# zzz5y/street_crafter

Measured on AMD Instinct MI355X. Metric: frames/sec @1M Gaussians 1920x1280 + PSNR vs ref; 1/2/4/8 MI355X, higher is better.
Workload: dtype f32

## Files before the change

### include/street_crafter_amd.h

```cpp
#ifndef STREET_CRAFTER_AMD_H
#define STREET_CRAFTER_AMD_H

#include <stddef.h>
#include <stdint.h>

#ifdef __cplusplus
extern "C" {
#endif

typedef void* sc_stream_t;

#define SC_OK 0
#define SC_EINVAL (-1)
#define SC_EWORKSPACE (-2)
#define SC_EUNSUPPORTED (-3)

const char* sc_version(void);
const char* sc_error_string(int code);
const char* sc_target_arch(void);
int sc_wait_i64(const int64_t* addr, int64_t value, int64_t timeout_us);

int sc_projection_fwd(const float* means, const float* quats, const float* scales,
                      const float* viewmats, const float* Ks, int C, int N, int width, int height,
                      float eps2d, float near_plane, float far_plane, float radius_clip,
// ... 42 lines not shown
int64_t sc_isect_split_seg_bound(int64_t n_records, int nsb);
int sc_isect_split_bins(const uint64_t* keys, int64_t n, uint64_t lo, uint64_t hi, int32_t* bins);
int sc_isect_split_plan(const uint32_t* bin_counts, int cap, int32_t* range_of_bin, int32_t* n_ranges);
int sc_isect_bin_sort(const float* means2d, const int32_t* radii, const float* depths, int C, int N,
                      int tile_size, int tile_width, int tile_height,
                      const int32_t* isect_offsets, const int64_t* meta_dev,
                      void* count_workspace ,
                      int64_t capacity, int64_t rec_capacity, int64_t super_capacity,
                      int64_t* isect_ids , int32_t* flatten_ids,
                      void* workspace, size_t ws_bytes, sc_stream_t stream);
int sc_isect_ids_rebuild(const int32_t* flatten_ids, const int32_t* isect_offsets, const float* depths,
                         int C, int N, int tile_width, int tile_height, int64_t n_isects,
                         int64_t* isect_ids, sc_stream_t stream);
int sc_isect_bin_reset_cursors(void* count_workspace, int64_t CN, int C, int tile_width, int tile_height,
                               sc_stream_t stream);

int sc_isect_offsets(const int64_t* isect_ids, int64_t n_isects, int C, int tile_width,
                     int tile_height, int32_t* offsets, sc_stream_t stream);

int sc_sh_fwd(int degree, const float* dirs, const float* coeffs, const uint8_t* masks,
              int64_t M, int K, float* colors, sc_stream_t stream);
int sc_sh_bwd(int degree, const float* dirs, const float* coeffs, const uint8_t* masks,
              int64_t M, int K, const float* v_colors, float* v_coeffs, float* v_dirs,
              sc_stream_t stream);

int sc_rasterize_fwd(const float* means2d, const float* conics, const float* colors,
                     const float* opacities, const float* backgrounds, const uint8_t* tile_masks,
                     int C, int N, int D, int width, int height, int tile_size,
                     int tile_width, int tile_height,
                     const int32_t* isect_offsets, const int32_t* flatten_ids, int64_t n_isects,
// ... 349 lines not shown
```

### street_crafter_amd/_lib.py

```python
from __future__ import annotations

import ctypes as C
import os

_HERE = os.path.dirname(os.path.abspath(__file__))
LIB_PATH = os.path.join(_HERE, "lib", "libstreet_crafter_hip.so")
DIAG_LIB_PATH = os.path.join(_HERE, "lib", "libstreet_crafter_hip_diag.so")

_lib = None
_path = LIB_PATH
_lock = __import__("threading").Lock()


def use_diagnostic_build(tag: str = ""):
    global _path
    want = DIAG_LIB_PATH.replace("_diag.so", f"_diag_{tag}.so") if tag else DIAG_LIB_PATH
    if _lib is not None and _path != want:
        raise RuntimeError("use_diagnostic_build() must be called before the library is first loaded")
    if not os.path.exists(want):
        raise ImportError(f"diagnostic library not built ({want} missing): "
                          "python -m street_crafter_amd.build --diag")
    _path = want

c_f32p = C.c_void_p
# ... 74 lines not shown
                                     c_i32p, c_i64p, c_i64p, C.c_int64, C.c_void_p, C.c_size_t, c_i32p, c_f32p, c_i32p,
                                     c_i32p, c_stream]),
    "sc_view_slots": (C.c_int, []),
    "sc_view_registry_words": (C.c_int, []),
    "sc_isect_bin_bucket_capacity": (C.c_int, []),
    "sc_isect_split_limits": (C.c_int, [c_i64p]),
    "sc_isect_split_seg_bound": (C.c_int64, [C.c_int64, C.c_int]),
    "sc_isect_split_bins": (C.c_int, [c_u64p, C.c_int64, C.c_uint64, C.c_uint64, c_i32p]),
    "sc_isect_split_plan": (C.c_int, [C.c_void_p, C.c_int, c_i32p, c_i32p]),
    "sc_isect_bin_sort": (C.c_int, [c_f32p, c_i32p, c_f32p, C.c_int, C.c_int, C.c_int, C.c_int, C.c_int,
                                    c_i32p, c_i64p, C.c_void_p, C.c_int64, C.c_int64, C.c_int64, c_i64p,
                                    c_i32p, C.c_void_p, C.c_size_t, c_stream]),
    "sc_isect_ids_rebuild": (C.c_int, [c_i32p, c_i32p, c_f32p, C.c_int, C.c_int, C.c_int, C.c_int, C.c_int64, c_i64p,
                                       c_stream]),
    "sc_isect_bin_reset_cursors": (C.c_int, [C.c_void_p, C.c_int64, C.c_int, C.c_int, C.c_int, c_stream]),
    "sc_isect_offsets": (C.c_int, [c_i64p, C.c_int64, C.c_int, C.c_int, C.c_int, c_i32p, c_stream]),
    "sc_sh_fwd": (C.c_int, [C.c_int, c_f32p, c_f32p, c_u8p, C.c_int64, C.c_int, c_f32p, c_stream]),
    "sc_sh_bwd": (C.c_int, [C.c_int, c_f32p, c_f32p, c_u8p, C.c_int64, C.c_int, c_f32p, c_f32p, c_f32p,
                            c_stream]),
    "sc_rasterize_fwd": (C.c_int, [c_f32p, c_f32p, c_f32p, c_f32p, c_f32p, c_u8p, C.c_int, C.c_int, C.c_int,
                                   C.c_int, C.c_int, C.c_int, C.c_int, C.c_int, c_i32p, c_i32p, C.c_int64,
                                   c_f32p, c_f32p, c_i32p, c_i32p, c_i32p, c_stream]),
    "sc_rasterize_fwd_ed": (C.c_int, [c_f32p, c_f32p, c_f32p, c_f32p, c_f32p, c_u8p, C.c_int, C.c_int, C.c_int,
                                      C.c_int, C.c_int, C.c_int, C.c_int, C.c_int, c_i32p, c_i32p, C.c_int64,
                                      c_f32p, c_f32p, c_i32p, c_i32p, c_stream]),
    "sc_rasterize_fwd_planar": (C.c_int, [c_f32p, c_f32p, c_f32p, c_f32p, c_f32p, c_u8p, C.c_int, C.c_int, C.c_int,
                                          C.c_int, C.c_int, C.c_int, C.c_int, C.c_int, c_i32p, c_i32p, C.c_int64,
                                          c_f32p, c_f32p, c_i32p, c_i32p, c_stream]),
    "sc_group_extents": (C.c_int, [c_i32p, c_i32p, C.c_int64, c_u8p, C.c_int, C.c_int, C.c_int, C.c_int, C.c_int,
                                   c_i32p, c_stream]),
# ... 135 lines not shown
    lib = C.CDLL(_path)
    for name, (res, args) in SIGNATURES.items():
        fn = getattr(lib, name)
        fn.restype = res
        fn.argtypes = args
    _lib = lib
    env_c, env_f = os.environ.get("SC_PROJ_CLAMP"), os.environ.get("SC_RADIUS_FLOOR")
    if env_c:
        if env_c not in ("symmetric", "asymmetric"):
            raise ValueError(f"SC_PROJ_CLAMP must be symmetric or asymmetric, got {env_c!r}")
        lib.sc_set_option(b"proj_clamp", 1 if env_c == "asymmetric" else 0)
    if env_f:
        if float(env_f) not in (0.01, 0.1):
            raise ValueError(f"SC_RADIUS_FLOOR must be 0.01 or 0.1, got {env_f!r}")
        lib.sc_set_option(b"radius_floor", 1 if float(env_f) == 0.1 else 0)
    return lib


FAST_PATH = os.path.join(_HERE, "lib", "_sc_fast.so")
_fast = None
_fast_enabled = True


def fast():
    global _fast
    if not _fast_enabled or _path != LIB_PATH:
        return None
    if _fast is None:
        load()
        with _lock:
# ... 65 lines not shown
```

### street_crafter_amd/csrc/capi.hip

```cpp
#include "raster_common.h"
#include <string.h>
#include <time.h>

#ifndef SC_ABI_HASH
#define SC_ABI_HASH "unhashed"
#endif
#ifdef SC_DIAG
extern "C" const char* sc_version(void) { return "street_crafter_amd 0.4.0 (gfx950, DIAGNOSTIC build) abi:" SC_ABI_HASH; }
#else
extern "C" const char* sc_version(void) { return "street_crafter_amd 0.4.0 (gfx950) abi:" SC_ABI_HASH; }
#endif

extern "C" const char* sc_target_arch(void) { return "gfx950"; }

extern "C" const char* sc_error_string(int code) {
    switch (code) {
        case SC_OK: return "ok";
        case SC_EINVAL: return "street_crafter_amd: invalid argument (size / null pointer / unsupported parameter)";
        case SC_EWORKSPACE: return "street_crafter_amd: workspace too small";
        case SC_EUNSUPPORTED: return "street_crafter_amd: unsupported configuration";
        default: break;
    }
    if (code > 0) return hipGetErrorString((hipError_t)code);
    return "street_crafter_amd: unknown error";
// ... 76 lines not shown
        if (value < 0 || value > 1) return SC_EINVAL;
        const int prev = g_sc_raster_map;
        g_sc_raster_map = value;
        return prev;
    }
    if (strcmp(key, "raster_hint_blend") == 0) {
        if (value < 0 || value > 4) return SC_EINVAL;
        const int prev = g_sc_raster_hint_blend;
        g_sc_raster_hint_blend = value;
        return prev;
    }
    if (strcmp(key, "raster_split") == 0) {
        if (value < 0 || value > 100) return SC_EINVAL;
        const int prev = g_sc_raster_split;
        g_sc_raster_split = value;
        return prev;
    }
    if (strcmp(key, "proj_clamp") == 0) {
        if (value < 0 || value > 1) return SC_EINVAL;
        const int prev = g_sc_proj_clamp;
        g_sc_proj_clamp = value;
        return prev;
    }
    if (strcmp(key, "radius_floor") == 0) {
        if (value < 0 || value > 1) return SC_EINVAL;
        const int prev = g_sc_radius_floor;
        g_sc_radius_floor = value;
        return prev;
    }
    if (strcmp(key, "point_raster_waves") == 0) {
// ... 232 lines not shown
```

### street_crafter_amd/csrc/isect_bin.hip

```cpp
#include "sc_common.h"

#pragma clang fp contract(off)

#include "isect_split_plan.h"

namespace {

constexpr int BIN_THREADS = 1024;
constexpr int BIN_GPT = 4;
constexpr int BIN_GPB = BIN_THREADS * BIN_GPT;
constexpr int CNT_GPT = 8;
constexpr int BIN_MAX_TILES = 36864;
constexpr int BIN_BIG = 32;
constexpr unsigned ID_MASK = 0x0fffffffu;
constexpr unsigned long long KEY_MASK = 0xffffffff0fffffffull;

struct Rect { int x0, x1, y0, y1; };

struct Geo {
    int tile_width, tile_height, T;
    int ss;
    int stw, sth, ST;
    int N;
};
// ... 405 lines not shown
        return;
    }
    const int cblock = (int)blockIdx.x - 3;
    unsigned* hist = lds;
    unsigned* gbase = lds + n_sbuckets;
    unsigned* cst = lds + 2 * n_sbuckets;
    {
        const int per = (n_sbuckets + BIN_THREADS - 1) / BIN_THREADS;
        const int beg = min((int)threadIdx.x * per, n_sbuckets), end = min(beg + per, n_sbuckets);
        long long sum = 0;
        for (int i = beg; i < end; ++i) sum += chist[i];
        long long tot;
        unsigned mx;
        long long run = block_scan_1024(sum, 0u, &tot, &mx, wave_tot, wave_max);
        for (int i = beg; i < end; ++i) { cst[i] = (unsigned)run; run += chist[i]; }
        if (cblock == 0 && threadIdx.x == 0) { cmeta[0] = tot; cmeta[1] = 0; }
    }
    for (int b = threadIdx.x; b < n_sbuckets; b += BIN_THREADS) hist[b] = 0;
    __syncthreads();
    const int64_t base = (int64_t)cblock * BIN_GPB;
    int cb[BIN_GPT];
    uint4 pay[BIN_GPT];
#pragma unroll
    for (int k = 0; k < BIN_GPT; ++k) {
        const int64_t i = base + (int64_t)k * BIN_THREADS + threadIdx.x;
        cb[k] = -1;
        pay[k] = make_uint4(0u, 0u, 0u, 0u);
        if (i < CN && tiles_per_gauss[i] > 0) {
            const float2 m = *reinterpret_cast<const float2*>(means2d + i * 2);
            const Rect r = tile_rect(m.x, m.y, radii[i], tile_size, g.tile_width, g.tile_height);
            const Rect s = super_rect(r, g.ss);
// ... 139 lines not shown
}

constexpr int SS_THREADS = 512;
constexpr int SS_WAVES = SS_THREADS / 64;
constexpr int SS_MAX_CAP = 3584;
constexpr int SS_RPT = SS_MAX_CAP / SS_THREADS;
constexpr int SS_NC = SS_THREADS;
constexpr int SS_SMALL_THREADS = 128;
constexpr int SS_SMALL_RPT = 8;
constexpr int SS_SMALL_CAP = SS_SMALL_THREADS * SS_SMALL_RPT;
constexpr int64_t BIG_MAX_SUPER = 220000;

struct Segment { int start, n, sb, heavy; int tb[4]; };

__device__ __forceinline__ unsigned long long rec_key60(uint2 r) {
    return ((unsigned long long)r.x << 28) | (unsigned long long)(r.y & ID_MASK);
}

template <int THREADS>
__device__ __forceinline__ void emit_tiles(const unsigned long long* __restrict__ S,
                                           const unsigned short* __restrict__ order, int n, int sb, const Geo& g,
                                           const int32_t* __restrict__ offsets, int n_tiles_total,
                                           int64_t n_isects, int tile_bits, const int* tb, unsigned long long* table,
                                           int64_t* __restrict__ isect_ids, int32_t* __restrict__ flatten_ids,
                                           unsigned* totals SC_DIAG_PARAM(dbg)) {
    constexpr int WAVES = THREADS / 64;
    const int t = threadIdx.x, lane = t & 63, wave = t >> 6;
    const int cam = sb / g.ST, srem = sb - cam * g.ST;
    const int sy = srem / g.stw, sx = srem - sy * g.stw;
    const int ntile = g.ss ? 4 : 1;
    const int rounds = (n + THREADS - 1) / THREADS;
// ... 46 lines not shown
                const int pos = tbase[k] + (int)((base >> (16 * k)) & 0xffffu) + __popcll(bal & sc_lanemask_lt());
                if (pos < tend[k]) {
                    if (isect_ids && !SC_DIAG_BIT(dbg, 16)) isect_ids[pos] = hi_key[k] | (long long)(key >> 32);
                    flatten_ids[pos] = (int32_t)((unsigned)key & ID_MASK);
                }
            }
        }
    }
}

__host__ __device__ inline size_t sort_lds_bytes(int cap, int threads = SS_THREADS) {
    const size_t table = (size_t)((cap + threads - 1) / threads + 1) * (threads / 64) * 8 + 64;
    return (size_t)cap * 10 + (size_t)((cap + 4) & ~1) * 4 + (size_t)threads * 4 + table + 16;
}

template <int THREADS, int RPT>
__device__ __forceinline__ void sort_segment(
    const uint2* __restrict__ recs, int n, int sb, const int* tb, int cap, const Geo& g,
    const int32_t* __restrict__ offsets, int n_tbuckets, int64_t n_isects, int tile_bits,
    unsigned char* smem, int64_t* __restrict__ isect_ids, int32_t* __restrict__ flatten_ids, unsigned* totals_out
    SC_DIAG_PARAM(dbg)) {
    constexpr int WAVES = THREADS / 64, NC = THREADS;
    unsigned long long* B = reinterpret_cast<unsigned long long*>(smem);
    unsigned short* order = reinterpret_cast<unsigned short*>(B + cap);
    unsigned* boff = reinterpret_cast<unsigned*>(order + cap);
    unsigned* coarse = boff + ((cap + 4) & ~1);
    unsigned long long* table = reinterpret_cast<unsigned long long*>(coarse + NC);
    unsigned* totals = reinterpret_cast<unsigned*>(reinterpret_cast<unsigned char*>(table) +
                                                   (size_t)((cap + THREADS - 1) / THREADS + 1) * WAVES * 8 + 64);
    __shared__ unsigned long long red_lo[WAVES], red_hi[WAVES];
    __shared__ unsigned red_sum[WAVES];
    const int t = threadIdx.x, lane = t & 63, wave = t >> 6;

    uint2 rec[RPT];
#pragma unroll
    for (int k = 0; k < RPT; ++k) {
// ... 15 lines not shown
    for (int o = 32; o >= 1; o >>= 1) {
        const unsigned long long l2 = (unsigned long long)__shfl_xor((long long)lo, o, 64);
        const unsigned long long h2 = (unsigned long long)__shfl_xor((long long)hi, o, 64);
        lo = l2 < lo ? l2 : lo;
        hi = h2 > hi ? h2 : hi;
    }
    if (lane == 0) { red_lo[wave] = lo; red_hi[wave] = hi; }
    __syncthreads();
    lo = red_lo[0]; hi = red_hi[0];
#pragma unroll
    for (int w = 1; w < WAVES; ++w) {
        lo = red_lo[w] < lo ? red_lo[w] : lo;
        hi = red_hi[w] > hi ? red_hi[w] : hi;
    }
    if (SC_DIAG_BIT(dbg, 4)) return;
    const double s1 = (double)NC / ((double)(hi - lo) + 1.0);
    auto level1 = [&](unsigned long long K, float& frac) -> int {
        const double p = (double)(K - lo) * s1;
        int c = (int)p;
        c = c < NC - 1 ? c : NC - 1;
        frac = (float)(p - (double)c);
        return c;
    };
#pragma unroll
    for (int k = 0; k < RPT; ++k) {
        if (t + k * THREADS < n) {
            float frac;
            atomicAdd(&coarse[level1(rec_key60(rec[k]), frac)], 1u);
        }
    }
    __syncthreads();
    {
        const unsigned c = coarse[t];
        const unsigned incl = (unsigned)sc_wave_incl_scan((int)c);
        if (lane == 63) red_sum[wave] = incl;
        __syncthreads();
        unsigned run = incl - c;
#pragma unroll
        for (int w = 0; w < WAVES; ++w) if (w < wave) run += red_sum[w];
        coarse[t] = c | (run << 16);
    }
    __syncthreads();
    if (SC_DIAG_BIT(dbg, 8)) return;
    auto fine_of = [&](unsigned long long K) -> int {
        float frac;
        const unsigned cs = coarse[level1(K, frac)];
        const int cnt = (int)(cs & 0xffffu);
        int f = (int)(frac * (float)cnt);
        f = f < cnt - 1 ? f : cnt - 1;
        return (int)(cs >> 16) + (f > 0 ? f : 0);
    };
    int fj[RPT];
#pragma unroll
    for (int k = 0; k < RPT; ++k) {
        fj[k] = 0;
        if (t + k * THREADS < n) {
            fj[k] = fine_of(rec_key60(rec[k]));
            atomicAdd(&boff[fj[k]], 1u);
        }
    }
    __syncthreads();
    {
        const int per = ((n + THREADS - 1) / THREADS) | 1;
        const int beg = min(t * per, n), end = min(beg + per, n);
        unsigned sum = 0;
        for (int i = beg; i < end; ++i) sum += boff[i];
        const unsigned incl = (unsigned)sc_wave_incl_scan((int)sum);
        __syncthreads();
        if (lane == 63) red_sum[wave] = incl;
        __syncthreads();
        unsigned run = incl - sum;
#pragma unroll
        for (int w = 0; w < WAVES; ++w) if (w < wave) run += red_sum[w];
        for (int i = beg; i < end; ++i) {
            const unsigned c = boff[i];
            boff[i] = run;
            run += c;
        }
    }
    __syncthreads();
    if (SC_DIAG_BIT(dbg, 32)) return;
#pragma unroll
    for (int k = 0; k < RPT; ++k) {
        if (t + k * THREADS < n) {
            const uint2 r = rec[k];
            const int f = fj[k];
            const unsigned slot = atomicAdd(&boff[f], 1u);
            B[slot] = ((unsigned long long)r.x << 32) | r.y;
            order[slot] = (unsigned short)f;
        }
    }
    __syncthreads();
    if (SC_DIAG_BIT(dbg, 2)) return;
    unsigned short bj[RPT];
#pragma unroll
    for (int k = 0; k < RPT; ++k) {
        const int p = t + k * THREADS;
        bj[k] = p < n ? order[p] : (unsigned short)0;
    }
    __syncthreads();
#pragma unroll
    for (int k = 0; k < RPT; ++k) {
        const int p = t + k * THREADS;
        if (p >= n) break;
        const unsigned long long kk = B[p] & KEY_MASK;
        const int j = bj[k];
        const unsigned beg = j > 0 ? boff[j - 1] : 0u, end = boff[j];
        unsigned r = beg;
        for (unsigned q = beg; q < end; ++q) r += ((B[q] & KEY_MASK) < kk) ? 1u : 0u;
        order[r] = (unsigned short)p;
    }
    __syncthreads();
    emit_tiles<THREADS>(B, order, n, sb, g, offsets, n_tbuckets, n_isects, tile_bits, tb, table, isect_ids,
                           flatten_ids, totals SC_DIAG_ARG(dbg));
    if (totals_out) {
        __syncthreads();
        if (t < 4) totals_out[t] = totals[t];
    }
}

__device__ __forceinline__ void sort_heavy_segment(
    const uint2* __restrict__ src, uint2* __restrict__ dst, int n, int sb, const int* tb_in, int cap, const Geo& g,
// ... 20 lines not shown
            const unsigned long long v = __hip_atomic_load(reinterpret_cast<const unsigned long long*>(dst + c0 + i),
                                                           __ATOMIC_RELAXED, __HIP_MEMORY_SCOPE_AGENT);
            B[i] = (v << 32) | (v >> 32);
        }
        __syncthreads();
        int tbl[4] = {tbr[0], tbr[1], tbr[2], tbr[3]};
        emit_tiles<SS_THREADS>(B, nullptr, m, sb, g, offsets, n_tbuckets, n_isects, tile_bits, tbl, table, isect_ids,
                               flatten_ids, tot SC_DIAG_ARG(0));
        __syncthreads();
        if (t < 4) tbr[t] += (int)tot[t];
        __syncthreads();
    }
}

template <int THREADS, int RPT>
__global__ __launch_bounds__(THREADS, 6) void super_sort_kernel(
    const uint2* __restrict__ records, uint2* __restrict__ records_rw, const uint2* __restrict__ temp,
    const Segment* __restrict__ segs, const unsigned* __restrict__ n_segs, int seg_bound,
    const int32_t* __restrict__ soffsets, int n_sbuckets, int n_tbuckets,
    Geo g, const int32_t* __restrict__ offsets, const int64_t* __restrict__ meta, int64_t capacity,
    int64_t rec_capacity, int64_t super_capacity, int tile_bits, int cap,
    int64_t* __restrict__ isect_ids, int32_t* __restrict__ flatten_ids SC_DIAG_PARAM(dbg)) {
    extern __shared__ __align__(16) unsigned char smem[];
    if (meta[0] > capacity || meta[2] > rec_capacity || meta[3] > super_capacity) return;
    __shared__ int tb_s[4];
    if (THREADS == SS_THREADS && (int)blockIdx.x < seg_bound) {
        if (blockIdx.x >= *n_segs) return;
        const Segment* sg = segs + blockIdx.x;
        if (threadIdx.x < 4) tb_s[threadIdx.x] = sg->tb[threadIdx.x];
        const int start = sg->start, sn = sg->n, ssb = sg->sb;
        __syncthreads();
        if (sg->heavy)
            sort_heavy_segment(temp + start, records_rw + start, sn, ssb, tb_s, cap, g, offsets, n_tbuckets,
                               meta[0], tile_bits, smem, isect_ids, flatten_ids);
        else
            sort_segment<SS_THREADS, SS_RPT>(temp + start, sn, ssb, tb_s, cap, g, offsets, n_tbuckets, meta[0], tile_bits,
                                             smem, isect_ids, flatten_ids, nullptr SC_DIAG_ARG(dbg));
        return;
    }
    const int sb = (int)blockIdx.x - seg_bound;
    const int s = soffsets[sb];
    const int e = (sb + 1 < n_sbuckets) ? soffsets[sb + 1] : (int)meta[2];
    const int n = e - s;
    if (n <= 0 || n > cap) return;
    if (threadIdx.x < 4) tb_s[threadIdx.x] = 0;
    __syncthreads();
    sort_segment<THREADS, RPT>(records + s, n, sb, tb_s, cap, g, offsets, n_tbuckets, meta[0], tile_bits, smem, isect_ids,
                               flatten_ids, nullptr SC_DIAG_ARG(dbg));
}

__global__ __launch_bounds__(256) void isect_ids_rebuild_kernel(
    const int32_t* __restrict__ flatten_ids, const int32_t* __restrict__ offsets, const float* __restrict__ depths,
    int n_tiles_total, int tiles_per_cam, int tile_bits, int64_t CN, int64_t n_isects, int64_t* __restrict__ isect_ids) {
    const int tflat = blockIdx.x;
    const int cam = tflat / tiles_per_cam, tile = tflat - cam * tiles_per_cam;
    int s = offsets[tflat];
    int e = (tflat + 1 < n_tiles_total) ? offsets[tflat + 1] : (int)n_isects;
    s = min(max(s, 0), (int)n_isects);
    e = min(max(e, s), (int)n_isects);
    const long long hi = ((long long)cam << (32 + tile_bits)) | ((long long)tile << 32);
    for (int k = s + (int)threadIdx.x; k < e; k += 256) {
        const int g = flatten_ids[k];
        const unsigned d = ((unsigned)g < (unsigned)CN) ? __float_as_uint(depths[g]) : 0u;
// ... 190 lines not shown
    L.nt_cells = C * (tile_height + 1) * (tile_width + 1);
    L.ns_cells = C * (L.g.sth + 1) * (L.g.stw + 1);
    const size_t nk = (size_t)L.nsb + 2;
    size_t o = 0;
    auto take = [&](size_t bytes) { const size_t at = o; o += sc_align_up(bytes, 256); return at; };
    L.dgrid_t = take((size_t)L.nt_cells * 4);
    L.dgrid_s = take((size_t)L.ns_cells * 4);
    L.chist = take(nk * 4);
    L.ccursor = take(nk * 4);
    L.rcursor = take((size_t)L.nsb * 4);
    L.nseg = take(4);
    L.scans_done = take(4);
    L.wstat = take(16);
    L.soffsets = take((size_t)L.nsb * 4);
    L.smeta = take(16);
    L.cmeta = take(16);
    L.whint = take((size_t)L.ntb * 4);
    L.sorted = take((size_t)(CN > 0 ? CN : 0) * 16);
    L.total = o;
    return L;
}

#include <mutex>
static hipError_t bin_attrs_once() {
    static std::mutex mu;
    static bool done[64] = {false};
    int dev = 0;
    hipError_t e = hipGetDevice(&dev);
    if (e != hipSuccess) return e;
    if (dev < 0 || dev >= 64) return hipErrorInvalidDevice;
    std::lock_guard<std::mutex> lock(mu);
// ... 37 lines not shown
    out[0] = BS_MAX_RANGES; out[1] = BIG_MAX_SUPER; out[2] = SS_MAX_CAP;
    out[3] = sp_light_max(SS_MAX_CAP); out[4] = sp_target(SS_MAX_CAP); out[5] = BS_NB;
    return SC_OK;
}

extern "C" int64_t sc_isect_split_seg_bound(int64_t n_records, int nsb) {
    return nsb < 0 ? (int64_t)SC_EINVAL : (int64_t)seg_bound_for(n_records, nsb);
}

extern "C" int sc_isect_split_bins(const uint64_t* keys, int64_t n, uint64_t lo, uint64_t hi, int32_t* bins) {
    if (n < 0 || hi < lo || (n > 0 && (!keys || !bins))) return SC_EINVAL;
    const double sc = sp_bin_scale(lo, hi);
    for (int64_t i = 0; i < n; ++i) {
        if (keys[i] < lo || keys[i] > hi) return SC_EINVAL;
        bins[i] = sp_bin_of(keys[i], lo, sc);
    }
    return SC_OK;
}

extern "C" int sc_isect_split_plan(const uint32_t* bin_counts, int cap, int32_t* range_of_bin, int32_t* n_ranges) {
    if (!bin_counts || !range_of_bin || !n_ranges || cap < 4) return SC_EINVAL;
    const int target = sp_target(cap), light_max = sp_light_max(cap);
    static_assert(sizeof(unsigned) == sizeof(uint32_t), "");
    unsigned gcnt[BS_NB], gmap[BS_NB], group_of_bin[BS_NB], rcnt[BS_NB], rstart[BS_NB];
    unsigned light = 0, H = 0;
    long long left = -1;
    int G = 0;
    for (int b = 0; b < BS_NB; ++b) {
        const unsigned c = bin_counts[b];
        const bool heavy = c > (unsigned)light_max;
// ... 92 lines not shown
    hipLaunchKernelGGL(center_scatter_kernel, dim3(grid + 3), dim3(BIN_THREADS), center_lds, s,
                       (const int32_t*)tiles_per_gauss, means2d, radii, CN, L.g, (float)tile_size, L.nsb,
                       depths, (const unsigned*)chist, ccursor, sorted, cmeta, jobs, scans_done, meta_dev,
                       meta_mirror, seq, (const unsigned*)whint, (const unsigned*)wstat, tile_order, L.ntb, staged,
                       g_sc_raster_split, g_sc_raster_bwd_split ? 0 : 1 SC_DIAG_ARG(g_sc_debug[1] >> 16));
    SC_LAUNCH_CHECK();
    return SC_OK;
}

extern "C" int sc_isect_bin_reset_cursors(void* count_workspace, int64_t CN, int C, int tile_width, int tile_height,
                                          sc_stream_t stream) {
    if (!count_workspace || C <= 0 || tile_width <= 0 || tile_height <= 0) return SC_EINVAL;
    if ((int64_t)C * tile_width * tile_height > BIN_MAX_TILES) return SC_EUNSUPPORTED;
    const BinLayout L = bin_layout(CN, C, 1, tile_width, tile_height);
    SC_HIP(hipMemsetAsync((unsigned char*)count_workspace + L.rcursor, 0, L.scans_done - L.rcursor, sc_s(stream)));
    return SC_OK;
}

extern "C" int sc_isect_ids_rebuild(const int32_t* flatten_ids, const int32_t* isect_offsets, const float* depths,
                                    int C, int N, int tile_width, int tile_height, int64_t n_isects,
                                    int64_t* isect_ids, sc_stream_t stream) {
    if (C < 0 || N < 0 || tile_width <= 0 || tile_height <= 0 || n_isects < 0 || n_isects > 0x7fffffffLL) return SC_EINVAL;
    if (C == 0 || n_isects == 0) return SC_OK;
    if (!flatten_ids || !isect_offsets || !depths || !isect_ids) return SC_EINVAL;
    const int64_t nb = (int64_t)C * tile_width * tile_height;
    if (nb > 0x7fffffffLL) return SC_EINVAL;
    hipLaunchKernelGGL(isect_ids_rebuild_kernel, dim3((unsigned)nb), dim3(256), 0, sc_s(stream), flatten_ids, isect_offsets,
                       depths, (int)nb, tile_width * tile_height, sc_bits_for((int64_t)tile_width * tile_height),
                       (int64_t)C * N, n_isects, isect_ids);
    SC_LAUNCH_CHECK();
// ... 38 lines not shown
    if (!few_huge)
        hipLaunchKernelGGL((bin_scatter_flat_kernel<FLAT_THREADS, 64>), dim3((unsigned)((CN + FLAT_THREADS - 1) / FLAT_THREADS)),
                           dim3(FLAT_THREADS), (size_t)L.nsb * 8 + 16 + (FLAT_THREADS / 64) * sizeof(FlatTab), s, sorted, cmeta,
                           L.g, L.nsb, soffsets, meta_dev, capacity, rec_capacity, super_capacity, cursor, records
                           SC_DIAG_ARG(g_sc_debug[0]));
    else {
        constexpr int gpb = FLAT_THREADS_SMALL / 64 * 16;
        hipLaunchKernelGGL((bin_scatter_flat_kernel<FLAT_THREADS_SMALL, 16>), dim3((unsigned)((CN + gpb - 1) / gpb)),
                           dim3(FLAT_THREADS_SMALL), (size_t)L.nsb * 8 + 16 + (FLAT_THREADS_SMALL / 64) * sizeof(FlatTab), s,
                           sorted, cmeta, L.g, L.nsb, soffsets, meta_dev, capacity, rec_capacity, super_capacity, cursor,
                           records SC_DIAG_ARG(g_sc_debug[0]));
    }
    SC_LAUNCH_CHECK();
    const int tile_bits = sc_bits_for(L.g.T);
    SC_HIP(bin_attrs_once());
    if (big) {
        const int bgrid = L.nsb;
        hipLaunchKernelGGL(big_split_kernel, dim3(bgrid), dim3(BS_THREADS), 0, s, (const uint2*)records, temp, segs,
                           n_segs, seg_bound, soffsets, L.nsb, meta_dev, capacity, rec_capacity, super_capacity, cap SC_DIAG_ARG(g_sc_debug[3]));
        SC_LAUNCH_CHECK();
    }
#define SC_LAUNCH_SORT(THREADSP, RPTP, GRID, LDSB, SEGB)                                                                      \
    hipLaunchKernelGGL((super_sort_kernel<THREADSP, RPTP>), dim3(GRID), dim3(THREADSP), LDSB, s,                              \
                       (const uint2*)records, records, (const uint2*)temp, (const Segment*)segs, (const unsigned*)n_segs, SEGB, \
                       soffsets, L.nsb, L.ntb, L.g, isect_offsets, meta_dev, capacity, rec_capacity, super_capacity, tile_bits,  \
                       cap, isect_ids, flatten_ids SC_DIAG_ARG(g_sc_debug[2]))
    if (!big && cap <= SS_SMALL_CAP)
        SC_LAUNCH_SORT(SS_SMALL_THREADS, SS_SMALL_RPT, (unsigned)L.nsb, sort_lds_bytes(cap, SS_SMALL_THREADS), 0);
    else
        SC_LAUNCH_SORT(SS_THREADS, SS_RPT, (unsigned)(seg_bound + L.nsb), sort_lds_bytes(cap), seg_bound);
#undef SC_LAUNCH_SORT
    SC_LAUNCH_CHECK();
    return SC_OK;
}
```

### street_crafter_amd/csrc/sc_common.h

```cpp
#pragma once
#include <hip/hip_runtime.h>
#include <stdint.h>
#include "../../include/street_crafter_amd.h"

#define SC_WAVE 64

#define SC_LAUNCH_CHECK()                                   \
    do {                                                    \
        hipError_t e__ = hipGetLastError();                 \
        if (e__ != hipSuccess) return (int)e__;             \
    } while (0)

#define SC_HIP(call)                                        \
    do {                                                    \
        hipError_t e__ = (call);                            \
        if (e__ != hipSuccess) return (int)e__;             \
    } while (0)

#ifdef SC_DIAG
extern int g_sc_debug[4];
#define SC_DIAG_PARAM(name) , int name
#define SC_DIAG_ARG(value) , (value)
#define SC_DIAG_BIT(name, mask) (((name) & (mask)) != 0)
__device__ __forceinline__ unsigned long long sc_diag_clock_raw() {
// ... 12 lines not shown
#else
#define SC_DIAG_PARAM(name)
#define SC_DIAG_ARG(value)
#define SC_DIAG_BIT(name, mask) false
#define SC_DIAG_CLOCK(on) 0ull
#define SC_DIAG_REALTIME(on) 0ull
#define SC_DIAG_DRAIN(on) do { } while (0)
#endif
extern "C" int sc_tile_order_len(int total_tiles);
constexpr int SC_VIEW_SLOTS = 8;
constexpr int SC_VIEW_REGISTRY_WORDS = 4 + 4 * SC_VIEW_SLOTS;
__host__ __device__ static inline int sc_clamp_view_slot(int v) { return v < 0 ? 0 : (v >= SC_VIEW_SLOTS ? SC_VIEW_SLOTS - 1 : v); }
extern int g_sc_raster_bwd_split;
extern int g_sc_raster_hint_blend;
extern int g_sc_raster_split;

static inline hipStream_t sc_s(sc_stream_t s) { return (hipStream_t)s; }

static inline size_t sc_align_up(size_t x, size_t a) { return (x + a - 1) / a * a; }

static inline int sc_bits_for(int64_t n) {
    int b = 0;
    while (n > 0) { ++b; n >>= 1; }
    return b < 1 ? 1 : b;
}

#ifdef __HIPCC__
__device__ __forceinline__ int sc_lane() { return (int)(threadIdx.x & 63); }

__device__ __forceinline__ int sc_wave_incl_scan(int v) {
// ... 34 lines not shown
```

### street_crafter_amd/isect.py

```python
from __future__ import annotations

import collections
import math
import os
import threading
import weakref
from typing import Optional, Tuple

import torch
from torch import Tensor

from . import _lib
from .lazy import LazyTensor as _LazyTensor


def _env_on(name: str, default: bool = True) -> bool:
    v = os.environ.get(name)
    return default if v is None or v == "" else v not in ("0", "false", "False", "off", "no")


class _Switches:
    __slots__ = ("tile_order", "lazy_ids", "view_slots", "packed_records", "defer_isect", "planar_out", "fused_train")

    def __init__(self):
# ... 15 lines not shown
    mi, mr, ms = map(max, zip(*history))
    ms_pred = ms + ms // 8 + 64
    if ms <= bucket_cap < ms_pred:
        ms_pred = bucket_cap
    return mi + mi // 8 + 4096, mr + mr // 8 + 4096, ms_pred


class _OperatorState:
    KEYS_MAX = 64

    def __init__(self):
        self.prediction, self.history, self.last_meta = {}, {}, {}
        self.history_len = 8
        self.tile_work, self.view_registry = {}, {}
        self.stats = {"calls": 0, "speculative_ok": 0, "exact_relaunch": 0}
        self.bucket_cap = {}
        self.sched_sizes = {}

    def tables(self):
        return (("predictions", self.prediction), ("history", self.history), ("last_meta", self.last_meta),
                ("tile_work", self.tile_work), ("view_registry", self.view_registry))

    def reset(self, idx=None) -> dict:
        dropped = {}
        for name, table in self.tables():
            keys = [k for k in table if idx is None or (k[0] if isinstance(k, tuple) else k) == idx]
            for k in keys:
                table.pop(k, None)
            dropped[name] = len(keys)
        return dropped
# ... 245 lines not shown
            if self.pred is not None:
                _lib.check(_lib.load().sc_isect_bin_reset_cursors(_p(self.ws0), C * N, C, tile_width, tile_height, st),
                           "sc_isect_bin_reset_cursors")
            if _stream(self.offsets) != st:
                with torch.cuda.stream(torch.cuda.ExternalStream(st, device=self.dev)):
                    rc = self.launch((n_isects, n_records, max_super))
                self.order_current_behind_producer()
            else:
                rc = self.launch((n_isects, n_records, max_super))
            if rc == -3:
                return None
            _lib.check(rc, "sc_isect_bin_sort")
        cap = _STATE.bucket_cap.get("v") or _STATE.bucket_cap.setdefault("v", int(_lib.load().sc_isect_bin_bucket_capacity()))
        _STATE.record(self.key, (n_isects, n_records, max_super), cap)
        self.flat, self.n_isects = self.fids[:n_isects], n_isects
        self.inputs = self.meta_dev = self.ws0 = None
        return n_isects

    def order_current_behind_producer(self):
        ev = torch.cuda.Event()
        ev.record(torch.cuda.ExternalStream(self.st, device=self.dev))
        torch.cuda.current_stream(self.dev).wait_event(ev)

    def fill_ids(self, buf):
        cur = _stream(buf)
        if cur != self.st:
            self.order_current_behind_producer()
        _lib.check(_lib.load().sc_isect_ids_rebuild(self.flat.data_ptr(), self.offsets.data_ptr(), self.depths.data_ptr(),
                                                    self.C, self.N, self.grid[1], self.grid[2], self.n_isects,
                                                    buf.data_ptr(), cur), "sc_isect_ids_rebuild")
# ... 95 lines not shown
```

Before: 3175.

## Add one-level distribution sort path with precomputed slots in segment sort

Segment sort now tries a single-level distribution bucketing (one bucket per record) first. It records each record's arrival index from the atomic increment so that scatter slots come from the prefix plus that index rather than a second atomic. It falls back to the two-level coarse/fine mapping when the largest bucket exceeds a small threshold. The intent is to skip the coarse histogram/scan pass and the per-record atomics in the scatter, which shortens the per-bucket insertion rank loop. Launch-bound occupancy hints are also raised, and optional path counters plus a host reference mapping are added.

```diff
diff --git a/include/street_crafter_amd.h b/include/street_crafter_amd.h
--- a/include/street_crafter_amd.h
+++ b/include/street_crafter_amd.h
@@ -80,6 +80,9 @@
                          int64_t* isect_ids, sc_stream_t stream);
 int sc_isect_bin_reset_cursors(void* count_workspace, int64_t CN, int C, int tile_width, int tile_height,
                                sc_stream_t stream);
+int sc_isect_bin_sort_paths(const void* count_workspace, int64_t CN, int C, int tile_width, int tile_height,
+                            int64_t* out , sc_stream_t stream);
+int sc_isect_sort_map(const uint64_t* keys, int64_t n, uint64_t lo, uint64_t hi, int levels, int nc, int32_t* fine);
 
 int sc_isect_offsets(const int64_t* isect_ids, int64_t n_isects, int C, int tile_width,
                      int tile_height, int32_t* offsets, sc_stream_t stream);
diff --git a/street_crafter_amd/_lib.py b/street_crafter_amd/_lib.py
--- a/street_crafter_amd/_lib.py
+++ b/street_crafter_amd/_lib.py
@@ -112,6 +112,8 @@
     "sc_isect_ids_rebuild": (C.c_int, [c_i32p, c_i32p, c_f32p, C.c_int, C.c_int, C.c_int, C.c_int, C.c_int64, c_i64p,
                                        c_stream]),
     "sc_isect_bin_reset_cursors": (C.c_int, [C.c_void_p, C.c_int64, C.c_int, C.c_int, C.c_int, c_stream]),
+    "sc_isect_bin_sort_paths": (C.c_int, [C.c_void_p, C.c_int64, C.c_int, C.c_int, C.c_int, c_i64p, c_stream]),
+    "sc_isect_sort_map": (C.c_int, [c_u64p, C.c_int64, C.c_uint64, C.c_uint64, C.c_int, C.c_int, c_i32p]),
     "sc_isect_offsets": (C.c_int, [c_i64p, C.c_int64, C.c_int, C.c_int, C.c_int, c_i32p, c_stream]),
     "sc_sh_fwd": (C.c_int, [C.c_int, c_f32p, c_f32p, c_u8p, C.c_int64, C.c_int, c_f32p, c_stream]),
     "sc_sh_bwd": (C.c_int, [C.c_int, c_f32p, c_f32p, c_u8p, C.c_int64, C.c_int, c_f32p, c_f32p, c_f32p,
@@ -277,6 +279,11 @@
         if float(env_f) not in (0.01, 0.1):
             raise ValueError(f"SC_RADIUS_FLOOR must be 0.01 or 0.1, got {env_f!r}")
         lib.sc_set_option(b"radius_floor", 1 if float(env_f) == 0.1 else 0)
+    env_l = os.environ.get("SC_ISECT_SORT_LEVELS")
+    if env_l:
+        if env_l not in ("0", "2"):
+            raise ValueError(f"SC_ISECT_SORT_LEVELS must be 0 or 2, got {env_l!r}")
+        lib.sc_set_option(b"isect_sort_levels", int(env_l))
     return lib
 
 
diff --git a/street_crafter_amd/csrc/capi.hip b/street_crafter_amd/csrc/capi.hip
--- a/street_crafter_amd/csrc/capi.hip
+++ b/street_crafter_amd/csrc/capi.hip
@@ -114,6 +114,18 @@
         if (value < 0 || value > 100) return SC_EINVAL;
         const int prev = g_sc_raster_split;
         g_sc_raster_split = value;
+        return prev;
+    }
+    if (strcmp(key, "isect_sort_levels") == 0) {
+        if (value != 0 && value != 2) return SC_EINVAL;
+        const int prev = g_sc_isect_sort_levels;
+        g_sc_isect_sort_levels = value;
+        return prev;
+    }
+    if (strcmp(key, "isect_sort_paths") == 0) {
+        if (value < 0 || value > 1) return SC_EINVAL;
+        const int prev = g_sc_isect_sort_paths;
+        g_sc_isect_sort_paths = value;
         return prev;
     }
     if (strcmp(key, "proj_clamp") == 0) {
diff --git a/street_crafter_amd/csrc/isect_bin.hip b/street_crafter_amd/csrc/isect_bin.hip
--- a/street_crafter_amd/csrc/isect_bin.hip
+++ b/street_crafter_amd/csrc/isect_bin.hip
@@ -3,6 +3,10 @@
 #pragma clang fp contract(off)
 
 #include "isect_split_plan.h"
+#include "isect_sort_map.h"
+
+int g_sc_isect_sort_levels = 0;
+int g_sc_isect_sort_paths = 0;
 
 namespace {
 
@@ -443,7 +447,7 @@
         unsigned mx;
         long long run = block_scan_1024(sum, 0u, &tot, &mx, wave_tot, wave_max);
         for (int i = beg; i < end; ++i) { cst[i] = (unsigned)run; run += chist[i]; }
-        if (cblock == 0 && threadIdx.x == 0) { cmeta[0] = tot; cmeta[1] = 0; }
+        if (cblock == 0 && threadIdx.x == 0) { cmeta[0] = tot; cmeta[1] = 0; cmeta[2] = 0; cmeta[3] = 0; }
     }
     for (int b = threadIdx.x; b < n_sbuckets; b += BIN_THREADS) hist[b] = 0;
     __syncthreads();
@@ -613,7 +617,7 @@
 struct Segment { int start, n, sb, heavy; int tb[4]; };
 
 __device__ __forceinline__ unsigned long long rec_key60(uint2 r) {
-    return ((unsigned long long)r.x << 28) | (unsigned long long)(r.y & ID_MASK);
+    return ((unsigned long long)(r.x >> 4) << 32) | (unsigned long long)((r.x << 28) | (r.y & ID_MASK));
 }
 
 template <int THREADS>
@@ -690,12 +694,15 @@
     return (size_t)cap * 10 + (size_t)((cap + 4) & ~1) * 4 + (size_t)threads * 4 + table + 16;
 }
 
+constexpr unsigned ONE_LEVEL_MAX = 16;
+
 template <int THREADS, int RPT>
 __device__ __forceinline__ void sort_segment(
     const uint2* __restrict__ recs, int n, int sb, const int* tb, int cap, const Geo& g,
     const int32_t* __restrict__ offsets, int n_tbuckets, int64_t n_isects, int tile_bits,
-    unsigned char* smem, int64_t* __restrict__ isect_ids, int32_t* __restrict__ flatten_ids, unsigned* totals_out
-    SC_DIAG_PARAM(dbg)) {
+    unsigned char* smem, int64_t* __restrict__ isect_ids, int32_t* __restrict__ flatten_ids, unsigned* totals_out,
+    int levels, unsigned long long* __restrict__ paths SC_DIAG_PARAM(dbg)) {
+    static_assert(THREADS <= SM_MAX_BINS && SS_MAX_CAP <= 4096, "coarse bin / bucket + arrival index share a word");
     constexpr int WAVES = THREADS / 64, NC = THREADS;
     unsigned long long* B = reinterpret_cast<unsigned long long*>(smem);
     unsigned short* order = reinterpret_cast<unsigned short*>(B + cap);
@@ -741,78 +748,106 @@
         hi = red_hi[w] > hi ? red_hi[w] : hi;
     }
     if (SC_DIAG_BIT(dbg, 4)) return;
-    const double s1 = (double)NC / ((double)(hi - lo) + 1.0);
-    auto level1 = [&](unsigned long long K, float& frac) -> int {
-        const double p = (double)(K - lo) * s1;
-        int c = (int)p;
-        c = c < NC - 1 ? c : NC - 1;
-        frac = (float)(p - (double)c);
-        return c;
-    };
-#pragma unroll
-    for (int k = 0; k < RPT; ++k) {
-        if (t + k * THREADS < n) {
-            float frac;
-            atomicAdd(&coarse[level1(rec_key60(rec[k]), frac)], 1u);
-        }
-    }
-    __syncthreads();
-    {
-        const unsigned c = coarse[t];
-        const unsigned incl = (unsigned)sc_wave_incl_scan((int)c);
-        if (lane == 63) red_sum[wave] = incl;
-        __syncthreads();
-        unsigned run = incl - c;
-#pragma unroll
-        for (int w = 0; w < WAVES; ++w) if (w < wave) run += red_sum[w];
-        coarse[t] = c | (run << 16);
-    }
-    __syncthreads();
-    if (SC_DIAG_BIT(dbg, 8)) return;
-    auto fine_of = [&](unsigned long long K) -> int {
-        float frac;
-        const unsigned cs = coarse[level1(K, frac)];
-        const int cnt = (int)(cs & 0xffffu);
-        int f = (int)(frac * (float)cnt);
-        f = f < cnt - 1 ? f : cnt - 1;
-        return (int)(cs >> 16) + (f > 0 ? f : 0);
-    };
-    int fj[RPT];
-#pragma unroll
-    for (int k = 0; k < RPT; ++k) {
-        fj[k] = 0;
-        if (t + k * THREADS < n) {
-            fj[k] = fine_of(rec_key60(rec[k]));
-            atomicAdd(&boff[fj[k]], 1u);
-        }
-    }
-    __syncthreads();
-    {
+    struct Word { unsigned v; } fj[RPT];
+    auto scan_boff = [&](unsigned keep_max) -> bool {
         const int per = ((n + THREADS - 1) / THREADS) | 1;
         const int beg = min(t * per, n), end = min(beg + per, n);
-        unsigned sum = 0;
-        for (int i = beg; i < end; ++i) sum += boff[i];
+        unsigned sum = 0, mx = 0;
+        for (int i = beg; i < end; ++i) {
+            const unsigned c = boff[i];
+            sum += c;
+            mx = c > mx ? c : mx;
+        }
         const unsigned incl = (unsigned)sc_wave_incl_scan((int)sum);
-        __syncthreads();
-        if (lane == 63) red_sum[wave] = incl;
+#pragma unroll
+        for (int o = 32; o >= 1; o >>= 1) {
+            const unsigned m2 = (unsigned)__shfl_xor((int)mx, o, 64);
+            mx = m2 > mx ? m2 : mx;
+        }
+        if (lane == 63) red_sum[wave] = incl | (mx << 16);
         __syncthreads();
         unsigned run = incl - sum;
-#pragma unroll
-        for (int w = 0; w < WAVES; ++w) if (w < wave) run += red_sum[w];
+        mx = 0;
+#pragma unroll
+        for (int w = 0; w < WAVES; ++w) {
+            const unsigned rs = red_sum[w];
+            if (w < wave) run += rs & 0xffffu;
+            mx = (rs >> 16) > mx ? (rs >> 16) : mx;
+        }
+        if (mx > keep_max) {
+            for (int i = beg; i < end; ++i) boff[i] = 0;
+            return false;
+        }
         for (int i = beg; i < end; ++i) {
             const unsigned c = boff[i];
             boff[i] = run;
             run += c;
         }
-    }
-    __syncthreads();
+        if (t == 0) boff[n] = (unsigned)n;
+        __syncthreads();
+        return true;
+    };
+#ifdef SC_DIAG
+    const unsigned one_level_max = ((dbg >> 8) & 0xff) ? (unsigned)((dbg >> 8) & 0xff) : ONE_LEVEL_MAX;
+#else
+    constexpr unsigned one_level_max = ONE_LEVEL_MAX;
+#endif
+    bool one_level = false;
+    if (levels != 2) {
+        const double s0 = sm_scale(lo, hi, n);
+#pragma unroll
+        for (int k = 0; k < RPT; ++k) {
+            fj[k].v = 0u;
+            if (t + k * THREADS < n) {
+                const unsigned f = (unsigned)sm_one_level(rec_key60(rec[k]), lo, s0, n);
+                fj[k].v = f | (atomicAdd(&boff[f], 1u) << 12);
+            }
+        }
+        __syncthreads();
+        one_level = scan_boff(one_level_max);
+        if (paths && t == 0) atomicAdd(&paths[one_level ? 0 : 1], 1ull);
+    }
+    if (!one_level) {
+        const double s1 = sm_scale(lo, hi, NC);
+#pragma unroll
+        for (int k = 0; k < RPT; ++k) {
+            fj[k].v = 0u;
+            if (t + k * THREADS < n) {
+                fj[k].v = sm_coarse(rec_key60(rec[k]), lo, s1, NC);
+                atomicAdd(&coarse[sm_coarse_bin(fj[k].v)], 1u);
+            }
+        }
+        __syncthreads();
+        {
+            const unsigned c = coarse[t];
+            const unsigned incl = (unsigned)sc_wave_incl_scan((int)c);
+            if (lane == 63) red_sum[wave] = incl;
+            __syncthreads();
+            unsigned run = incl - c;
+#pragma unroll
+            for (int w = 0; w < WAVES; ++w) if (w < wave) run += red_sum[w];
+            coarse[t] = c | (run << 16);
+        }
+        __syncthreads();
+        if (SC_DIAG_BIT(dbg, 8)) return;
+#pragma unroll
+        for (int k = 0; k < RPT; ++k) {
+            if (t + k * THREADS < n) {
+                const unsigned cs = coarse[sm_coarse_bin(fj[k].v)];
+                const unsigned f = (unsigned)sm_fine(fj[k].v, cs & 0xffffu, cs >> 16);
+                fj[k].v = f | (atomicAdd(&boff[f], 1u) << 12);
+            }
+        }
+        __syncthreads();
+        scan_boff(~0u);
+    }
     if (SC_DIAG_BIT(dbg, 32)) return;
 #pragma unroll
     for (int k = 0; k < RPT; ++k) {
         if (t + k * THREADS < n) {
             const uint2 r = rec[k];
-            const int f = fj[k];
-            const unsigned slot = atomicAdd(&boff[f], 1u);
+            const unsigned f = fj[k].v & 0xfffu;
+            const unsigned slot = boff[f] + (fj[k].v >> 12);
             B[slot] = ((unsigned long long)r.x << 32) | r.y;
             order[slot] = (unsigned short)f;
         }
@@ -832,7 +867,7 @@
         if (p >= n) break;
         const unsigned long long kk = B[p] & KEY_MASK;
         const int j = bj[k];
-        const unsigned beg = j > 0 ? boff[j - 1] : 0u, end = boff[j];
+        const unsigned beg = boff[j], end = boff[j + 1];
         unsigned r = beg;
         for (unsigned q = beg; q < end; ++q) r += ((B[q] & KEY_MASK) < kk) ? 1u : 0u;
         order[r] = (unsigned short)p;
@@ -883,13 +918,14 @@
 }
 
 template <int THREADS, int RPT>
-__global__ __launch_bounds__(THREADS, 6) void super_sort_kernel(
+__global__ __launch_bounds__(THREADS, THREADS == SS_THREADS ? 8 : 7) void super_sort_kernel(
     const uint2* __restrict__ records, uint2* __restrict__ records_rw, const uint2* __restrict__ temp,
     const Segment* __restrict__ segs, const unsigned* __restrict__ n_segs, int seg_bound,
     const int32_t* __restrict__ soffsets, int n_sbuckets, int n_tbuckets,
     Geo g, const int32_t* __restrict__ offsets, const int64_t* __restrict__ meta, int64_t capacity,
     int64_t rec_capacity, int64_t super_capacity, int tile_bits, int cap,
-    int64_t* __restrict__ isect_ids, int32_t* __restrict__ flatten_ids SC_DIAG_PARAM(dbg)) {
+    int64_t* __restrict__ isect_ids, int32_t* __restrict__ flatten_ids, int levels,
+    unsigned long long* __restrict__ paths SC_DIAG_PARAM(dbg)) {
     extern __shared__ __align__(16) unsigned char smem[];
     if (meta[0] > capacity || meta[2] > rec_capacity || meta[3] > super_capacity) return;
     __shared__ int tb_s[4];
@@ -904,7 +940,7 @@
                                meta[0], tile_bits, smem, isect_ids, flatten_ids);
         else
             sort_segment<SS_THREADS, SS_RPT>(temp + start, sn, ssb, tb_s, cap, g, offsets, n_tbuckets, meta[0], tile_bits,
-                                             smem, isect_ids, flatten_ids, nullptr SC_DIAG_ARG(dbg));
+                                             smem, isect_ids, flatten_ids, nullptr, levels, paths SC_DIAG_ARG(dbg));
         return;
     }
     const int sb = (int)blockIdx.x - seg_bound;
@@ -915,7 +951,7 @@
     if (threadIdx.x < 4) tb_s[threadIdx.x] = 0;
     __syncthreads();
     sort_segment<THREADS, RPT>(records + s, n, sb, tb_s, cap, g, offsets, n_tbuckets, meta[0], tile_bits, smem, isect_ids,
-                               flatten_ids, nullptr SC_DIAG_ARG(dbg));
+                               flatten_ids, nullptr, levels, paths SC_DIAG_ARG(dbg));
 }
 
 __global__ __launch_bounds__(256) void isect_ids_rebuild_kernel(
@@ -1136,7 +1172,7 @@
     L.wstat = take(16);
     L.soffsets = take((size_t)L.nsb * 4);
     L.smeta = take(16);
-    L.cmeta = take(16);
+    L.cmeta = take(32);
     L.whint = take((size_t)L.ntb * 4);
     L.sorted = take((size_t)(CN > 0 ? CN : 0) * 16);
     L.total = o;
@@ -1204,6 +1240,29 @@
     for (int64_t i = 0; i < n; ++i) {
         if (keys[i] < lo || keys[i] > hi) return SC_EINVAL;
         bins[i] = sp_bin_of(keys[i], lo, sc);
+    }
+    return SC_OK;
+}
+
+extern "C" int sc_isect_sort_map(const uint64_t* keys, int64_t n, uint64_t lo, uint64_t hi, int levels, int nc,
+                                 int32_t* fine) {
+    if (n < 0 || n > SS_MAX_CAP || hi < lo || (levels != 1 && levels != 2) || (n > 0 && (!keys || !fine))) return SC_EINVAL;
+    if (levels == 2 && nc != SS_THREADS && nc != SS_SMALL_THREADS) return SC_EINVAL;
+    for (int64_t i = 0; i < n; ++i)
+        if (keys[i] < lo || keys[i] > hi) return SC_EINVAL;
+    if (levels == 1) {
+        const double s0 = sm_scale(lo, hi, (int)n);
+        for (int64_t i = 0; i < n; ++i) fine[i] = sm_one_level(keys[i], lo, s0, (int)n);
+        return SC_OK;
+    }
+    unsigned count[SS_THREADS] = {0u}, first[SS_THREADS];
+    const double s1 = sm_scale(lo, hi, nc);
+    for (int64_t i = 0; i < n; ++i) ++count[sm_coarse_bin(sm_coarse(keys[i], lo, s1, nc))];
+    unsigned run = 0;
+    for (int c = 0; c < nc; ++c) { first[c] = run; run += count[c]; }
+    for (int64_t i = 0; i < n; ++i) {
+        const unsigned cq = sm_coarse(keys[i], lo, s1, nc);
+        fine[i] = sm_fine(cq, count[sm_coarse_bin(cq)], first[sm_coarse_bin(cq)]);
     }
     return SC_OK;
 }
@@ -1326,6 +1385,16 @@
     if ((int64_t)C * tile_width * tile_height > BIN_MAX_TILES) return SC_EUNSUPPORTED;
     const BinLayout L = bin_layout(CN, C, 1, tile_width, tile_height);
     SC_HIP(hipMemsetAsync((unsigned char*)count_workspace + L.rcursor, 0, L.scans_done - L.rcursor, sc_s(stream)));
+    return SC_OK;
+}
+
+extern "C" int sc_isect_bin_sort_paths(const void* count_workspace, int64_t CN, int C, int tile_width, int tile_height,
+                                       int64_t* out, sc_stream_t stream) {
+    if (!count_workspace || !out || C <= 0 || tile_width <= 0 || tile_height <= 0) return SC_EINVAL;
+    if ((int64_t)C * tile_width * tile_height > BIN_MAX_TILES) return SC_EUNSUPPORTED;
+    const BinLayout L = bin_layout(CN, C, 1, tile_width, tile_height);
+    SC_HIP(hipMemcpyAsync(out, (const unsigned char*)count_workspace + L.cmeta + 16, 16, hipMemcpyDeviceToHost, sc_s(stream)));
+    SC_HIP(hipStreamSynchronize(sc_s(stream)));
     return SC_OK;
 }
 
@@ -1394,6 +1463,8 @@
     SC_LAUNCH_CHECK();
     const int tile_bits = sc_bits_for(L.g.T);
     SC_HIP(bin_attrs_once());
+    const int sort_levels = g_sc_isect_sort_levels;
+    unsigned long long* sort_paths = g_sc_isect_sort_paths ? (unsigned long long*)(cws + L.cmeta) + 2 : nullptr;
     if (big) {
         const int bgrid = L.nsb;
         hipLaunchKernelGGL(big_split_kernel, dim3(bgrid), dim3(BS_THREADS), 0, s, (const uint2*)records, temp, segs,
@@ -1404,7 +1475,7 @@
     hipLaunchKernelGGL((super_sort_kernel<THREADSP, RPTP>), dim3(GRID), dim3(THREADSP), LDSB, s,                              \
                        (const uint2*)records, records, (const uint2*)temp, (const Segment*)segs, (const unsigned*)n_segs, SEGB, \
                        soffsets, L.nsb, L.ntb, L.g, isect_offsets, meta_dev, capacity, rec_capacity, super_capacity, tile_bits,  \
-                       cap, isect_ids, flatten_ids SC_DIAG_ARG(g_sc_debug[2]))
+                       cap, isect_ids, flatten_ids, sort_levels, sort_paths SC_DIAG_ARG(g_sc_debug[2]))
     if (!big && cap <= SS_SMALL_CAP)
         SC_LAUNCH_SORT(SS_SMALL_THREADS, SS_SMALL_RPT, (unsigned)L.nsb, sort_lds_bytes(cap, SS_SMALL_THREADS), 0);
     else
diff --git a/street_crafter_amd/csrc/isect_sort_map.h b/street_crafter_amd/csrc/isect_sort_map.h
--- /dev/null
+++ b/street_crafter_amd/csrc/isect_sort_map.h
@@ -0,0 +1,35 @@
+#pragma once
+#include <stdint.h>
+
+#if !defined(__HIPCC__) && !defined(__host__)
+#define __host__
+#define __device__
+#endif
+
+constexpr int SM_FRAC_BITS = 23;
+constexpr int SM_BIN_BITS = 32 - SM_FRAC_BITS;
+constexpr int SM_MAX_BINS = 1 << SM_BIN_BITS;
+
+__host__ __device__ inline double sm_scale(unsigned long long lo, unsigned long long hi, int buckets) {
+    return (double)buckets / ((double)(hi - lo) + 1.0);
+}
+
+__host__ __device__ inline int sm_one_level(unsigned long long K, unsigned long long lo, double scale, int n) {
+    const int f = (int)((double)(K - lo) * scale);
+    return f < n - 1 ? f : n - 1;
+}
+
+__host__ __device__ inline unsigned sm_coarse(unsigned long long K, unsigned long long lo, double scale, int nc) {
+    const double p = (double)(K - lo) * scale;
+    int c = (int)p;
+    c = c < nc - 1 ? c : nc - 1;
+    unsigned q = (unsigned)((p - (double)c) * (double)(1u << SM_FRAC_BITS));
+    q = q < (1u << SM_FRAC_BITS) - 1u ? q : (1u << SM_FRAC_BITS) - 1u;
+    return ((unsigned)c << SM_FRAC_BITS) | q;
+}
+__host__ __device__ inline int sm_coarse_bin(unsigned cq) { return (int)(cq >> SM_FRAC_BITS); }
+
+__host__ __device__ inline int sm_fine(unsigned cq, unsigned count, unsigned first) {
+    const unsigned q = cq << SM_BIN_BITS;
+    return (int)(first + (unsigned)(((unsigned long long)q * count) >> 32));
+}
diff --git a/street_crafter_amd/csrc/sc_common.h b/street_crafter_amd/csrc/sc_common.h
--- a/street_crafter_amd/csrc/sc_common.h
+++ b/street_crafter_amd/csrc/sc_common.h
@@ -50,6 +50,8 @@
 extern int g_sc_raster_bwd_split;
 extern int g_sc_raster_hint_blend;
 extern int g_sc_raster_split;
+extern int g_sc_isect_sort_levels;
+extern int g_sc_isect_sort_paths;
 
 static inline hipStream_t sc_s(sc_stream_t s) { return (hipStream_t)s; }
 
diff --git a/street_crafter_amd/isect.py b/street_crafter_amd/isect.py
--- a/street_crafter_amd/isect.py
+++ b/street_crafter_amd/isect.py
@@ -1,6 +1,7 @@
 from __future__ import annotations
 
 import collections
+import ctypes
 import math
 import os
 import threading
@@ -53,6 +54,7 @@
         self.history_len = 8
         self.tile_work, self.view_registry = {}, {}
         self.stats = {"calls": 0, "speculative_ok": 0, "exact_relaunch": 0}
+        self.sort_paths = None
         self.bucket_cap = {}
         self.sched_sizes = {}
 
@@ -328,6 +330,11 @@
         cap = _STATE.bucket_cap.get("v") or _STATE.bucket_cap.setdefault("v", int(_lib.load().sc_isect_bin_bucket_capacity()))
         _STATE.record(self.key, (n_isects, n_records, max_super), cap)
         self.flat, self.n_isects = self.fids[:n_isects], n_isects
+        if _STATE.sort_paths is not None:
+            out = (ctypes.c_int64 * 2)()
+            _lib.check(_lib.load().sc_isect_bin_sort_paths(_p(self.ws0), C * N, C, tile_width, tile_height,
+                                                           ctypes.addressof(out), st), "sc_isect_bin_sort_paths")
+            _STATE.sort_paths.append((int(out[0]), int(out[1])))
         self.inputs = self.meta_dev = self.ws0 = None
         return n_isects
 
```

Result: no change. 3188 (median of 2 runs) (+0.4%).
